# tylerlum/Vine_Robot_IsaacGymEnvs

Hardware: AMD Instinct MI355X
Metric: env-steps/sec Vine5LinkMovingBase 16384 envs per GPU (higher is better)
Workload: dtype f32 (env step, rollout inference); update: fp16 GEMM operands and backward-only saved activations (gates, saved cell states, dG, dh), f32 accumulate / recurrent state / heads / loss / optimiser, device-side GradScaler loss scaling (mixed_precision: True = the reference YAML's value, PY:53); rollout

## Files before the change

### vine_robot_isaacgymenvs_amd/csrc/ppo_kernels.hip

```cpp

#include <hip/hip_runtime.h>

#include <cstdio>
#include <cstdlib>

#include "../../include/vine.h"
#include "../../include/vine_ppo.h"
#include "vine_policy_head.h"
#include "vine_ppo_formulas.h"

namespace {

__device__ __forceinline__ float4 ld4(const float* p) { return *reinterpret_cast<const float4*>(p); }
__device__ __forceinline__ void st4(float* p, float4 v) { *reinterpret_cast<float4*>(p) = v; }

typedef unsigned short lp16_t;
typedef __attribute__((__vector_size__(2 * sizeof(float)))) float f32x2_hw;
#ifdef VINE_LP_BF16
typedef __bf16 lp16_hw;
#define VINE_LP16_NAME "bf16"
#define MFMA_LP16_BUILTIN __builtin_amdgcn_mfma_f32_16x16x32_bf16
#define DS_READ_TR16_B64 __builtin_amdgcn_ds_read_tr16_b64_v4bf16
typedef __bf16 lp16_tr_hw;
#define LP16_MAX 3.3895314e38f
// ... 286 lines not shown
    }
    __syncthreads();
    const int q = threadIdx.x & 15, rg = threadIdx.x >> 4;
    const int j = u0 + 4 * q;
    float bv[4][4];
#pragma unroll
    for (int g = 0; g < 4; ++g) {
        const float4 bb = ld4(bias + g * H + j);
        bv[g][0] = bb.x; bv[g][1] = bb.y; bv[g][2] = bb.z; bv[g][3] = bb.w;
    }
#pragma unroll
    for (int p = 0; p < 4; ++p) {
        const int r = rg + 16 * p;
        const long long b = (long long)blockIdx.x * 64 + r;
        const float keep = keep_pre[p], kn = kn_pre[p];
        float pre[4][4];
#pragma unroll
        for (int g = 0; g < 4; ++g) {
            const float4 a = *reinterpret_cast<const float4*>(&gt[r * GP + g * 64 + 4 * q]);
            pre[g][0] = a.x + bv[g][0]; pre[g][1] = a.y + bv[g][1]; pre[g][2] = a.z + bv[g][2]; pre[g][3] = a.w + bv[g][3];
            if (igates) {
                const float4 ig = ld4(igates + b * ig_stride + g * H + j);
                pre[g][0] += ig.x; pre[g][1] += ig.y; pre[g][2] += ig.z; pre[g][3] += ig.w;
            }
        }
        const float4 cp = cpre[p];
        const float cpv[4] = {cp.x, cp.y, cp.z, cp.w};
        float gi[4], gf[4], gg[4], go[4], cn[4], hn[4];
#pragma unroll
        for (int u = 0; u < 4; ++u)
            lstm_cell(pre[0][u], pre[1][u], pre[2][u], pre[3][u], keep * cpv[u], gi[u], gf[u], gg[u], go[u], cn[u], hn[u]);
        st4(c_out + b * H + j, make_float4(cn[0], cn[1], cn[2], cn[3]));
        st4(h_out + b * h_stride + j, make_float4(hn[0], hn[1], hn[2], hn[3]));
        if (hp_next) st4(hp_next + b * hp_stride + j, make_float4(kn * hn[0], kn * hn[1], kn * hn[2], kn * hn[3]));
        if (gates_act) {
            lp16_t* ga = gates_act + b * 4LL * H;
            st4(ga + 0 * H + j, make_float4(gi[0], gi[1], gi[2], gi[3]));
            st4(ga + 1 * H + j, make_float4(gf[0], gf[1], gf[2], gf[3]));
            st4(ga + 2 * H + j, make_float4(gg[0], gg[1], gg[2], gg[3]));
            st4(ga + 3 * H + j, make_float4(go[0], go[1], go[2], go[3]));
        }
    }
}

__device__ __forceinline__ float dpp_i2f(int x) { return __builtin_bit_cast(float, x); }
__device__ __forceinline__ int dpp_f2i(float x) { return __builtin_bit_cast(int, x); }
constexpr int SEQ_ROWS = 32;
constexpr int LDS_SKEW = 16;
constexpr int SEQ_FWD_NC = 11;
constexpr int SEQ_H = 256;
#ifndef SEQ_BWD_RING
#define SEQ_BWD_RING 8
#endif

__device__ __forceinline__ void seq_barrier() {
    asm volatile("s_waitcnt lgkmcnt(0)\n\ts_barrier" ::: "memory");
}

__global__ __launch_bounds__(256) void lstm_tile_weights_kernel(const lp16_t* __restrict__ src, long long ld, int H, int ksteps,
                                                                int nj, int transposed, lp16_t* __restrict__ dst) {
    const long long chunks = (long long)(H / 32) * ksteps * nj * 64;
    for (long long c = (long long)blockIdx.x * blockDim.x + threadIdx.x; c < chunks; c += (long long)gridDim.x * blockDim.x) {
        const int lane = (int)(c & 63);
        long long r = c >> 6;
        const int j = (int)(r % nj); r /= nj;
        const int kk = (int)(r % ksteps);
        const int w = (int)(r / ksteps);
        const int ut = nj == 8 ? (j & 1) : j, g = nj == 8 ? (j >> 1) : 0;
        const int unit = 32 * w + 8 * ((lane & 15) >> 2) + 4 * ut + (lane & 3);
        const int k0 = 32 * kk + 8 * (lane >> 4);
        uint4 v;
        if (!transposed) {
            v = *reinterpret_cast<const uint4*>(src + (long long)(g * H + unit) * ld + k0);
        } else {
            lp16_t e[8];
#pragma unroll
            for (int i = 0; i < 8; ++i) e[i] = src[(long long)(k0 + i) * ld + unit];
            v.x = e[0] | ((unsigned)e[1] << 16); v.y = e[2] | ((unsigned)e[3] << 16);
            v.z = e[4] | ((unsigned)e[5] << 16); v.w = e[6] | ((unsigned)e[7] << 16);
        }
        *reinterpret_cast<uint4*>(dst + c * 8) = v;
    }
}

typedef __attribute__((__vector_size__(4 * sizeof(unsigned)))) unsigned u32x4_t;
__device__ __forceinline__ uint4 seq_load_frag(__amdgpu_buffer_rsrc_t rsrc, int voffset, int soffset) {
    const u32x4_t v = __builtin_amdgcn_raw_buffer_load_b128(rsrc, voffset, soffset, 0);
    return make_uint4(v[0], v[1], v[2], v[3]);
}
__device__ __forceinline__ uint4 pack_lp16x8(const float (&v)[8]) {
    uint4 r;
    r.x = f2lp2(v[0], v[1]); r.y = f2lp2(v[2], v[3]); r.z = f2lp2(v[4], v[5]); r.w = f2lp2(v[6], v[7]);
    return r;
}

#ifdef SPLIT_TIMING
__device__ unsigned long long mlp_split_t[4096 * 16];
#endif
#if defined(SPLIT_TIMING) && defined(BWD_STAMPS)
#define BSTAMP(i)                                                                                                       \
    if ((threadIdx.x & 63) == 0) {                                                                                      \
        mlp_split_t[((blockIdx.x * 8 + (threadIdx.x >> 6)) & 4095) * 16 + 2 * (i)] = __builtin_amdgcn_s_memtime();      \
        mlp_split_t[((blockIdx.x * 8 + (threadIdx.x >> 6)) & 4095) * 16 + 2 * (i) + 1] = __builtin_amdgcn_s_memrealtime(); \
    }
#else
#define BSTAMP(i)
#endif
#ifdef SEQ_TIMING
__device__ unsigned long long seq_t[256 * 8 * 16];
#endif
template <int KS1, int RING, typename CT, typename HT, int NC>
__device__ __forceinline__ void lstm_seq_fwd_body(
    int T, long long B, const lp16_t* __restrict__ x, long long ldx, lp16_t* hp, long long hp_stride,
    const uint4* __restrict__ Wt, const float* __restrict__ bias, const float* __restrict__ c0,
    const unsigned char* __restrict__ done, HT* __restrict__ h_out, CT* __restrict__ c_all,
    lp16_t* __restrict__ gates, int ablate, float* __restrict__ c_last, const float* __restrict__ h0) {
    constexpr int H = SEQ_H, KSTEPS = KS1 + 8, KX = 32 * KS1, NF = KSTEPS * 8;
    constexpr int XP = KX + LDS_SKEW, HP = H + LDS_SKEW;
    static_assert(NF % RING == 0, "the ring must close on a step boundary");
    extern __shared__ __attribute__((aligned(16))) unsigned char seqf_lds[];
    float* bias_l = reinterpret_cast<float*>(seqf_lds);
    lp16_t (*hl)[SEQ_ROWS * HP] = reinterpret_cast<lp16_t (*)[SEQ_ROWS * HP]>(seqf_lds + 4 * H * sizeof(float));
    lp16_t (*xs)[SEQ_ROWS * XP] = reinterpret_cast<lp16_t (*)[SEQ_ROWS * XP]>(seqf_lds + 4 * H * sizeof(float) +
                                                                            2 * SEQ_ROWS * HP * sizeof(lp16_t));
    const int tid = threadIdx.x, lane = tid & 63;
    const int w = __builtin_amdgcn_readfirstlane(tid >> 6);
    const int col = lane & 15, lq = lane >> 4;
    const long long b0 = (long long)blockIdx.x * SEQ_ROWS;
    const int U0 = 32 * w + 8 * lq;
    const __amdgpu_buffer_rsrc_t wrsrc = __builtin_amdgcn_make_buffer_rsrc(
        const_cast<char*>(reinterpret_cast<const char*>(Wt) + (long long)w * NF * 1024), 0, NF * 1024, 0x00020000);
    const int wlane = lane * 16;
#define SEQ_WFRAG(f) seq_load_frag(wrsrc, wlane, (f) * 1024)
    uint4 ring[RING];
#pragma unroll
    for (int i = 0; i < RING; ++i) ring[i] = SEQ_WFRAG(i);
    static_assert(NC <= NF - RING && NC <= RING, "cached fragments are re-requested from the tail of the previous step only");
    uint4* wcache = reinterpret_cast<uint4*>(seqf_lds + 4 * H * sizeof(float) + 2 * SEQ_ROWS * HP * sizeof(lp16_t) +
                                             (size_t)T * SEQ_ROWS * XP * sizeof(lp16_t)) + (w * NC) * 64 + lane;
    {
        for (int p = tid; p < T * SEQ_ROWS * (KX / 8); p += 512) {
            const int tt = p / (SEQ_ROWS * (KX / 8)), q = p - tt * (SEQ_ROWS * (KX / 8));
            const int r = q / (KX / 8), c8 = q - r * (KX / 8);
            *reinterpret_cast<uint4*>(&xs[tt][r * XP + 8 * c8]) =
                *reinterpret_cast<const uint4*>(x + ((b0 + r) * T + tt) * ldx + 8 * c8);
        }
        for (int p = tid; p < SEQ_ROWS * (H / 8); p += 512) {
            const int r = p >> 5, c8 = p & 31;
            uint4 hv;
            if (h0) {
                const float keep0 = (done && done[(b0 + r) * T]) ? 0.0f : 1.0f;
                const float4 a = ld4(h0 + (b0 + r) * H + 8 * c8), b = ld4(h0 + (b0 + r) * H + 8 * c8 + 4);
                const float v[8] = {keep0 * a.x, keep0 * a.y, keep0 * a.z, keep0 * a.w, keep0 * b.x, keep0 * b.y, keep0 * b.z, keep0 * b.w};
                hv = pack_lp16x8(v);
                if (sizeof(HT) == 2) {
                    const float u8[8] = {a.x, a.y, a.z, a.w, b.x, b.y, b.z, b.w};
                    *reinterpret_cast<uint4*>(reinterpret_cast<lp16_t*>(h_out) + (b0 + r) * (T + 1) * H + 8 * c8) = pack_lp16x8(u8);
                } else {
                    *reinterpret_cast<uint4*>(hp + (b0 + r) * hp_stride + 8 * c8) = hv;
                }
            } else {
                hv = *reinterpret_cast<const uint4*>(hp + (b0 + r) * hp_stride + 8 * c8);
            }
            *reinterpret_cast<uint4*>(&hl[0][r * HP + 8 * c8]) = hv;
        }
        for (int p = tid; p < H; p += 512) st4(&bias_l[4 * p], ld4(bias + 4 * p));
    }
    float c[2][8];
    unsigned dmask[2];
#pragma unroll
    for (int rt = 0; rt < 2; ++rt) {
        const long long b = b0 + 16 * rt + col;
        const float4 a = ld4(c0 + b * H + U0), bb = ld4(c0 + b * H + U0 + 4);
        c[rt][0] = a.x; c[rt][1] = a.y; c[rt][2] = a.z; c[rt][3] = a.w;
        c[rt][4] = bb.x; c[rt][5] = bb.y; c[rt][6] = bb.z; c[rt][7] = bb.w;
        unsigned m = 0;
        if (done)
            for (int t = 0; t < T; ++t) m |= (done[b * T + t] ? 1u : 0u) << t;
        dmask[rt] = m;
    }
#pragma unroll 1
    for (int t = 0; t < T; ++t) {
#ifdef SEQ_TIMING
        if (lane == 0 && t < 4) seq_t[(blockIdx.x * 8 + w) * 16 + 4 * t + 0] = wall_clock64();
#endif
        if (t == 0) seq_barrier();
        const lp16_t* xb = xs[t];
        const lp16_t* hb = hl[t & 1];
        lp16_t* hnext = hl[(t + 1) & 1];
        const bool last = t == T - 1;
// ... 37 lines not shown
#endif
                    const int fn = (f + RING) % NF;
                    if (fn < NC && f + RING >= NF) ring[slot] = wcache[fn * 64];
                    else ring[slot] = SEQ_WFRAG(fn);
                }
                __builtin_amdgcn_sched_barrier(0);
            }
        }
#ifdef SEQ_TIMING
        if (lane == 0 && t < 4) seq_t[(blockIdx.x * 8 + w) * 16 + 4 * t + 2] = wall_clock64();
#endif
#pragma unroll
        for (int rt = 0; rt < 2; ++rt) {
            const long long b = b0 + 16 * rt + col;
            const float keep = ((dmask[rt] >> t) & 1u) ? 0.0f : 1.0f;
            const float kn = ((dmask[rt] >> (t + 1)) & 1u) ? 0.0f : 1.0f;
            CT* cp = c_all + ((long long)(t + 1) * B + b) * H + U0;
            float* cl = c_last + b * H + U0;
            HT* hpo = h_out + (sizeof(HT) == 2 ? b * (T + 1) + t + 1 : b * T + t) * H + U0;
            uint2 lo[6];
#pragma unroll
            for (int ut = 0; ut < 2; ++ut) {
                const float4 bi = *reinterpret_cast<const float4*>(&bias_l[0 * H + U0 + 4 * ut]);
                const float4 bf_ = *reinterpret_cast<const float4*>(&bias_l[1 * H + U0 + 4 * ut]);
                const float4 bg = *reinterpret_cast<const float4*>(&bias_l[2 * H + U0 + 4 * ut]);
                const float4 bo = *reinterpret_cast<const float4*>(&bias_l[3 * H + U0 + 4 * ut]);
                const float bv[4][4] = {{bi.x, bi.y, bi.z, bi.w}, {bf_.x, bf_.y, bf_.z, bf_.w}, {bg.x, bg.y, bg.z, bg.w},
                                        {bo.x, bo.y, bo.z, bo.w}};
                float gi[4], gf[4], gg[4], go[4], hn[4];
#pragma unroll
                for (int u = 0; u < 4; ++u)
                    lstm_cell(acc[0][ut][rt][u] + bv[0][u], acc[1][ut][rt][u] + bv[1][u], acc[2][ut][rt][u] + bv[2][u],
                              acc[3][ut][rt][u] + bv[3][u], keep * c[rt][4 * ut + u], gi[u], gf[u], gg[u], go[u],
                              c[rt][4 * ut + u], hn[u]);
                if (!(ablate & 1)) {
                    const float4 cv = make_float4(c[rt][4 * ut], c[rt][4 * ut + 1], c[rt][4 * ut + 2], c[rt][4 * ut + 3]);
                    if (sizeof(CT) == 2 && last) st4(cl + 4 * ut, cv);
                    else st4(cp + 4 * ut, cv);
                    if (sizeof(HT) == 4) st4(hpo + 4 * ut, make_float4(hn[0], hn[1], hn[2], hn[3]));
                }
                uint2 pk[6];
                pk[5] = make_uint2(f2lp2(hn[0], hn[1]), f2lp2(hn[2], hn[3]));
                pk[0] = make_uint2(f2lp2(gi[0], gi[1]), f2lp2(gi[2], gi[3]));
                pk[1] = make_uint2(f2lp2(gf[0], gf[1]), f2lp2(gf[2], gf[3]));
                pk[2] = make_uint2(f2lp2(gg[0], gg[1]), f2lp2(gg[2], gg[3]));
                pk[3] = make_uint2(f2lp2(go[0], go[1]), f2lp2(go[2], go[3]));
                pk[4] = make_uint2(f2lp2(kn * hn[0], kn * hn[1]), f2lp2(kn * hn[2], kn * hn[3]));
                if (ut == 0) {
#pragma unroll
                    for (int a = 0; a < 6; ++a) lo[a] = pk[a];
                } else {
                    if (sizeof(HT) == 2 && !(ablate & 1))
                        *reinterpret_cast<uint4*>(hpo) = make_uint4(lo[5].x, lo[5].y, pk[5].x, pk[5].y);
                    if (gates && !(ablate & 1)) {
                        lp16_t* ga = gates + ((long long)t * B + b) * 4 * H + U0;
#pragma unroll
                        for (int g = 0; g < 4; ++g)
                            *reinterpret_cast<uint4*>(ga + g * H) = make_uint4(lo[g].x, lo[g].y, pk[g].x, pk[g].y);
                    }
                    if (!last) {
                        const uint4 hm = make_uint4(lo[4].x, lo[4].y, pk[4].x, pk[4].y);
                        *reinterpret_cast<uint4*>(&hnext[(16 * rt + col) * HP + U0]) = hm;
                        if (sizeof(HT) == 4 && !(ablate & 1))
                            *reinterpret_cast<uint4*>(hp + b * hp_stride + (long long)(t + 1) * H + U0) = hm;
                    }
                }
            }
        }
#ifdef SEQ_TIMING
        if (lane == 0 && t < 4) seq_t[(blockIdx.x * 8 + w) * 16 + 4 * t + 3] = wall_clock64();
#endif
    }
}
template <int KS1, int RING, typename CT, typename HT, int NC>
__global__ __launch_bounds__(512) void lstm_seq_fwd_kernel(
    int T, long long B, const lp16_t* __restrict__ x, long long ldx, lp16_t* hp, long long hp_stride,
    const uint4* __restrict__ Wt, const float* __restrict__ bias, const float* __restrict__ c0,
    const unsigned char* __restrict__ done, HT* __restrict__ h_out, CT* __restrict__ c_all,
    lp16_t* __restrict__ gates, int ablate, float* __restrict__ c_last, const float* __restrict__ h0) {
    lstm_seq_fwd_body<KS1, RING, CT, HT, NC>(T, B, x, ldx, hp, hp_stride, Wt, bias, c0, done, h_out, c_all, gates, ablate, c_last,
                                             h0);
}

__device__ __forceinline__ float dpp_row_sum16(float v) {
    float s = v + dpp_i2f(__builtin_amdgcn_update_dpp(0, dpp_f2i(v), 0x111, 0xf, 0xf, true));
    s += dpp_i2f(__builtin_amdgcn_update_dpp(0, dpp_f2i(v), 0x112, 0xf, 0xf, true));
    s += dpp_i2f(__builtin_amdgcn_update_dpp(0, dpp_f2i(v), 0x113, 0xf, 0xf, true));
    s += dpp_i2f(__builtin_amdgcn_update_dpp(0, dpp_f2i(s), 0x114, 0xf, 0xe, true));
    s += dpp_i2f(__builtin_amdgcn_update_dpp(0, dpp_f2i(s), 0x118, 0xf, 0xc, true));
    return s;
}
__device__ __forceinline__ void unpack_lp16x8(uint4 r, float (&v)[8]) {
    unpack2(r.x, v[0], v[1]); unpack2(r.y, v[2], v[3]); unpack2(r.z, v[4], v[5]); unpack2(r.w, v[6], v[7]);
}

template <int RING, typename CT, typename GT>
__device__ __forceinline__ void lstm_seq_bwd_body(
    int T, long long B, const GT* __restrict__ g_out, const uint4* __restrict__ Wt, const lp16_t* __restrict__ gates,
    const CT* __restrict__ c_all, const float* __restrict__ c0, const unsigned char* __restrict__ done,
    lp16_t* __restrict__ dG, float* __restrict__ bias_partial, int ablate, const float* __restrict__ c_last) {
    constexpr int H = SEQ_H, K = 4 * H, KSTEPS = K / 32, NF = KSTEPS * 2;
    constexpr int PITCH = K + LDS_SKEW;
    static_assert(NF % RING == 0, "the ring must close on a step boundary");
    extern __shared__ __attribute__((aligned(16))) unsigned char seq_lds[];
    lp16_t (*dgl)[SEQ_ROWS * PITCH] = reinterpret_cast<lp16_t (*)[SEQ_ROWS * PITCH]>(seq_lds);
    const int tid = threadIdx.x, lane = tid & 63;
    const int w = __builtin_amdgcn_readfirstlane(tid >> 6);
    const int col = lane & 15, lq = lane >> 4;
    const long long b0 = (long long)blockIdx.x * SEQ_ROWS;
    const int U0 = 32 * w + 8 * lq;
    const __amdgpu_buffer_rsrc_t wrsrc = __builtin_amdgcn_make_buffer_rsrc(
        const_cast<char*>(reinterpret_cast<const char*>(Wt) + (long long)w * NF * 1024), 0, NF * 1024, 0x00020000);
    const int wlane = lane * 16;
    uint4 ring[RING];
#pragma unroll
    for (int i = 0; i < RING; ++i) ring[i] = SEQ_WFRAG(i);
    unsigned dmask[2];
    float dcarry[2][8], cnew[2][8], bsum[4][8];
#pragma unroll
    for (int rt = 0; rt < 2; ++rt) {
        const long long b = b0 + 16 * rt + col;
        unsigned m = 0;
        if (done)
            for (int t = 0; t < T; ++t) m |= (done[b * T + t] ? 1u : 0u) << t;
        dmask[rt] = m;
        float4 a, bb;
        if (sizeof(CT) == 2) { a = ld4(c_last + b * H + U0); bb = ld4(c_last + b * H + U0 + 4); }
        else { a = ld4(c_all + ((long long)T * B + b) * H + U0); bb = ld4(c_all + ((long long)T * B + b) * H + U0 + 4); }
        cnew[rt][0] = a.x; cnew[rt][1] = a.y; cnew[rt][2] = a.z; cnew[rt][3] = a.w;
        cnew[rt][4] = bb.x; cnew[rt][5] = bb.y; cnew[rt][6] = bb.z; cnew[rt][7] = bb.w;
#pragma unroll
        for (int e = 0; e < 8; ++e) dcarry[rt][e] = 0.0f;
    }
#pragma unroll
    for (int g = 0; g < 4; ++g)
#pragma unroll
        for (int e = 0; e < 8; ++e) bsum[g][e] = 0.0f;
    auto step = [&](const int t, auto first_c) __attribute__((always_inline)) {
        constexpr bool first = decltype(first_c)::value;
        float4 go4[2][2], cp4[2][2];
        uint4 gpk[2][4];
#define SEQ_BWD_LOAD(rt)                                                                                   \
        {                                                                                                  \
            const long long b_ = b0 + 16 * (rt) + col;                                                     \
            const GT* gp_ = g_out + (b_ * T + t) * H + U0;                                                 \
            go4[rt][0] = ld4(gp_); go4[rt][1] = ld4(gp_ + 4);                                              \
            if (t == 0) {                                                                                  \
                cp4[rt][0] = ld4(c0 + b_ * H + U0); cp4[rt][1] = ld4(c0 + b_ * H + U0 + 4);                \
            } else {                                                                                       \
                const CT* cpp_ = c_all + ((long long)t * B + b_) * H + U0;                                 \
                cp4[rt][0] = ld4(cpp_); cp4[rt][1] = ld4(cpp_ + 4);                                        \
            }                                                                                              \
            const lp16_t* ga_ = gates + ((long long)t * B + b_) * 4 * H + U0;                              \
            _Pragma("unroll") for (int g = 0; g < 4; ++g) gpk[rt][g] = *reinterpret_cast<const uint4*>(ga_ + g * H); \
        }
        SEQ_BWD_LOAD(0)
        f32x4_t acc[2][2];
#pragma unroll
        for (int ut = 0; ut < 2; ++ut)
#pragma unroll
            for (int rt = 0; rt < 2; ++rt) acc[ut][rt] = f32x4_t{0.0f, 0.0f, 0.0f, 0.0f};
        if (!first) {
            seq_barrier();
            const lp16_t* xb = dgl[(t + 1) & 1];
            if (t == T - 2) { BSTAMP(5) }
#pragma unroll
            for (int kk = 0; kk < KSTEPS; ++kk) {
                const lp16x8_t a0 = *reinterpret_cast<const lp16x8_t*>(xb + col * PITCH + 32 * kk + 8 * lq);
                const lp16x8_t a1 = *reinterpret_cast<const lp16x8_t*>(xb + (16 + col) * PITCH + 32 * kk + 8 * lq);
#pragma unroll
                for (int j = 0; j < 2; ++j) {
                    const int f = kk * 2 + j, slot = f % RING;
                    const lp16x8_t wf = __builtin_bit_cast(lp16x8_t, ring[slot]);
                    acc[j][0] = MFMA_LP16(wf, a0, acc[j][0]);
                    acc[j][1] = MFMA_LP16(wf, a1, acc[j][1]);
                    if (!(ablate & 2)) ring[slot] = SEQ_WFRAG((f + RING) % NF);
                    __builtin_amdgcn_sched_barrier(0);
                }
            }
            if (t == T - 2) { BSTAMP(6) }
        }
        lp16_t* dgn = dgl[t & 1];
        SEQ_BWD_LOAD(1)
#undef SEQ_BWD_LOAD
#pragma unroll
        for (int rt = 0; rt < 2; ++rt) {
            const long long b = b0 + 16 * rt + col;
            const float keep = ((dmask[rt] >> t) & 1u) ? 0.0f : 1.0f;
            const float keep_n = ((dmask[rt] >> (t + 1)) & 1u) ? 0.0f : 1.0f;
            lp16_t* dgp = dG + (b * T + t) * 4 * H + U0;
            uint2 lo[4];
#pragma unroll
            for (int ut = 0; ut < 2; ++ut) {
                float gi[4], gf[4], gg[4], go[4];
                const unsigned ia = ut ? gpk[rt][0].z : gpk[rt][0].x, ib = ut ? gpk[rt][0].w : gpk[rt][0].y;
                const unsigned fa = ut ? gpk[rt][1].z : gpk[rt][1].x, fb = ut ? gpk[rt][1].w : gpk[rt][1].y;
                const unsigned ga_ = ut ? gpk[rt][2].z : gpk[rt][2].x, gb_ = ut ? gpk[rt][2].w : gpk[rt][2].y;
                const unsigned oa = ut ? gpk[rt][3].z : gpk[rt][3].x, ob = ut ? gpk[rt][3].w : gpk[rt][3].y;
                unpack2(ia, gi[0], gi[1]); unpack2(ib, gi[2], gi[3]);
                unpack2(fa, gf[0], gf[1]); unpack2(fb, gf[2], gf[3]);
                unpack2(ga_, gg[0], gg[1]); unpack2(gb_, gg[2], gg[3]);
                unpack2(oa, go[0], go[1]); unpack2(ob, go[2], go[3]);
                const float gout[4] = {go4[rt][ut].x, go4[rt][ut].y, go4[rt][ut].z, go4[rt][ut].w};
                const float cp[4] = {cp4[rt][ut].x, cp4[rt][ut].y, cp4[rt][ut].z, cp4[rt][ut].w};
                float di[4], df[4], dg[4], dout[4];
#pragma unroll
                for (int u = 0; u < 4; ++u) {
                    const int e = 4 * ut + u;
                    float dh = gout[u];
                    if (!first) dh += keep_n * acc[ut][rt][u];
                    float dc = first ? 0.0f : keep_n * dcarry[rt][e];
                    if (!first) asm volatile("" : "+v"(dc));
                    lstm_cell_bwd(dh, dc, cnew[rt][e], keep * cp[u], gi[u], gf[u], gg[u], go[u], di[u], df[u], dg[u], dout[u],
                                  dcarry[rt][e]);
                    cnew[rt][e] = cp[u];
                    bsum[0][e] += di[u]; bsum[1][e] += df[u]; bsum[2][e] += dg[u]; bsum[3][e] += dout[u];
                }
                uint2 pk[4];
                pk[0] = make_uint2(f2lp2(di[0], di[1]), f2lp2(di[2], di[3]));
                pk[1] = make_uint2(f2lp2(df[0], df[1]), f2lp2(df[2], df[3]));
                pk[2] = make_uint2(f2lp2(dg[0], dg[1]), f2lp2(dg[2], dg[3]));
                pk[3] = make_uint2(f2lp2(dout[0], dout[1]), f2lp2(dout[2], dout[3]));
                if (ut == 0) {
#pragma unroll
                    for (int g = 0; g < 4; ++g) lo[g] = pk[g];
                } else {
                    lp16_t* row = dgn + (16 * rt + col) * PITCH + U0;
#pragma unroll
                    for (int g = 0; g < 4; ++g) {
                        const uint4 v = make_uint4(lo[g].x, lo[g].y, pk[g].x, pk[g].y);
                        if (!(ablate & 1)) *reinterpret_cast<uint4*>(dgp + g * H) = v;
                        if (t > 0) *reinterpret_cast<uint4*>(row + g * H) = v;
                    }
                }
            }
// ... 2601 lines not shown
    __syncthreads();
    if (threadIdx.x == 0) {
        const unsigned t = atomicAdd(ticket, 1u);
        is_last = t == gridDim.x - 1;
        if (is_last) *ticket = 0;
    }
    __syncthreads();
    if (is_last) {
        __threadfence();
        ppo_loss_finalize((int)gridDim.x, A, n, loss_partial, logstd, critic_coef, entropy_coef, bounds_coef, stats,
                          grad_logstd, grad_mu_bias, grad_value_bias, kl_out, logstd_grad_accum, S);
    }
}
template <int NH, int NP, typename DXT, typename XT>
__global__ __launch_bounds__(512) void ln_heads_loss_kernel(
    long long n, const XT* __restrict__ x, int xT, const float* __restrict__ gamma, const float* __restrict__ beta, float eps,
    const float* __restrict__ w, const float* __restrict__ wb, const float* __restrict__ logstd,
    const float* __restrict__ actions, const float* __restrict__ old_neglogp, const float* __restrict__ adv,
    const float* __restrict__ old_values, const float* __restrict__ returns, const float* old_mu, const float* old_sigma,
    float e_clip, int clip_value, float critic_coef, float entropy_coef, float bounds_coef, float soft_bound,
    float* __restrict__ heads, DXT* __restrict__ dx, float* __restrict__ ln_partial, float* loss_partial,
    float* __restrict__ stats, float* __restrict__ grad_logstd, float* __restrict__ grad_mu_bias,
    float* __restrict__ grad_value_bias, float* __restrict__ kl_out, float* __restrict__ logstd_grad_accum, float* mu_store,
    float* sigma_store, const float* __restrict__ loss_scale, float* __restrict__ found_inf, unsigned int* ticket,
    int defer) {
    __shared__ float red_s[8 * (2 + NH) * 256];
    __shared__ float lred_s[8 * PPO_LOSS_ROW];
    ln_heads_loss_body<NH, NP, DXT, XT>(red_s, lred_s, n, x, xT, gamma, beta, eps, w, wb, logstd, actions, old_neglogp, adv,
                                        old_values, returns, old_mu, old_sigma, e_clip, clip_value, critic_coef, entropy_coef,
                                        bounds_coef, soft_bound, heads, dx, ln_partial, loss_partial, stats, grad_logstd,
                                        grad_mu_bias, grad_value_bias, kl_out, logstd_grad_accum, mu_store, sigma_store,
                                        loss_scale, found_inf, ticket, defer);
}

struct TrunkPhasesArgs {
    long long B; int T;
    const lp16_t* x; long long ldx; const uint4* w_tiled; const float* bias; const float* c0; const float* h0;
    const unsigned char* done; lp16_t* h_out; lp16_t* c_all; lp16_t* gates; float* c_last; int ablate;
    const float* gamma; const float* beta; float eps; const float* w; const float* wb; const float* logstd;
    const float* actions; const float* old_neglogp; const float* adv; const float* old_values; const float* returns;
    const float* old_mu; const float* old_sigma; float e_clip; int clip_value; float critic_coef, entropy_coef, bounds_coef,
        soft_bound;
    float* heads; lp16_t* dx; float* ln_partial; float* loss_partial; float* stats; float* grad_logstd; float* grad_mu_bias;
    float* grad_value_bias; float* kl_out; float* logstd_grad_accum; float* mu_store; float* sigma_store;
    const float* loss_scale; float* found_inf;
    const uint4* w_hh_tiled; lp16_t* dG; float* bias_partial;
    const lp16_t* wt0; long long ldw0; const lp16_t* wt1; long long ldw1; const lp16_t* wt2; long long ldw2;
    const lp16_t* a3; long long a3_stride; const lp16_t* a2; const lp16_t* a1; float alpha;
    lp16_t* gz3; lp16_t* gz2; lp16_t* gz1; float* part3; float* part2; float* part1;
};
__global__ __launch_bounds__(512) void trunk_phases_kernel(const TrunkPhasesArgs a) {
    extern __shared__ __attribute__((aligned(16))) unsigned char trunk_lds[];
    TRUNK_STAMP(0)
    lstm_seq_fwd_body<3, 22, lp16_t, lp16_t, SEQ_FWD_NC>(a.T, a.B, a.x, a.ldx, nullptr, 0, a.w_tiled, a.bias, a.c0, a.done, a.h_out, a.c_all,
                                                 a.gates, a.ablate, a.c_last, a.h0);
    __syncthreads();
    TRUNK_STAMP(1)
    ln_heads_loss_body<3, 4, lp16_t, lp16_t>(reinterpret_cast<float*>(trunk_lds),
                                             reinterpret_cast<float*>(trunk_lds) + 8 * 5 * 256, a.B * a.T, a.h_out, a.T, a.gamma,
                                             a.beta, a.eps, a.w, a.wb, a.logstd, a.actions, a.old_neglogp, a.adv, a.old_values,
                                             a.returns, a.old_mu, a.old_sigma, a.e_clip, a.clip_value, a.critic_coef,
                                             a.entropy_coef, a.bounds_coef, a.soft_bound, a.heads, a.dx, a.ln_partial,
                                             a.loss_partial, a.stats, a.grad_logstd, a.grad_mu_bias, a.grad_value_bias, a.kl_out,
                                             a.logstd_grad_accum, a.mu_store, a.sigma_store, a.loss_scale, a.found_inf, nullptr,
                                             1 );
    __syncthreads();
    TRUNK_STAMP(2)
    lstm_seq_bwd_body<SEQ_BWD_RING, lp16_t, lp16_t>(a.T, a.B, a.dx, a.w_hh_tiled, a.gates, a.c_all, a.c0, a.done, a.dG,
                                                    a.bias_partial, a.ablate, a.c_last);
    __syncthreads();
    TRUNK_STAMP(3)
    mlp3_bwd_elu_mfma_body<64, 128, 256, 8, 8>(a.B * a.T, a.dG, 4 * SEQ_H, a.wt0, a.ldw0, a.wt1, a.ldw1, a.wt2, a.ldw2, a.a3,
                                              a.a3_stride, a.a2, a.a1, a.alpha, a.gz3, a.gz2, a.gz1, a.part3, a.part2, a.part1);
    TRUNK_STAMP(4)
}
#undef LHL_COL
#undef LHL_ROW

#define GRAD_SQNORM_MAX_PARTS 256
template <int CTRL, int ROW_MASK, int BANK_MASK>
__device__ __forceinline__ double dpp_f64(double v) {
    const unsigned long long b = __builtin_bit_cast(unsigned long long, v);
    const unsigned lo = (unsigned)__builtin_amdgcn_update_dpp(0, (int)(unsigned)b, CTRL, ROW_MASK, BANK_MASK, true);
    const unsigned hi = (unsigned)__builtin_amdgcn_update_dpp(0, (int)(unsigned)(b >> 32), CTRL, ROW_MASK, BANK_MASK, true);
    return __builtin_bit_cast(double, ((unsigned long long)hi << 32) | lo);
}
__device__ __forceinline__ double wave_sum_f64(double v) {
    double s = v + dpp_f64<0x111, 0xf, 0xf>(v);
    s += dpp_f64<0x112, 0xf, 0xf>(v);
    s += dpp_f64<0x113, 0xf, 0xf>(v);
    s += dpp_f64<0x114, 0xf, 0xe>(s);
    s += dpp_f64<0x118, 0xf, 0xc>(s);
    s += dpp_f64<0x142, 0xa, 0xf>(s);
    s += dpp_f64<0x143, 0xc, 0xf>(s);
    const unsigned long long b = __builtin_bit_cast(unsigned long long, s);
    const unsigned lo = (unsigned)__builtin_amdgcn_readlane((int)(unsigned)b, 63);
    const unsigned hi = (unsigned)__builtin_amdgcn_readlane((int)(unsigned)(b >> 32), 63);
    return __builtin_bit_cast(double, ((unsigned long long)hi << 32) | lo);
}

__global__ __launch_bounds__(256) void grad_sqnorm_kernel(long long n, const float* __restrict__ g,
                                                          double* __restrict__ partial) {
    __shared__ double ws[4];
    const long long n4 = n >> 2, stride = (long long)gridDim.x * 256;
    double a0 = 0.0, a1 = 0.0, a2 = 0.0, a3 = 0.0;
    for (long long i = (long long)blockIdx.x * 256 + threadIdx.x; i < n4; i += 2 * stride) {
        const bool more = i + stride < n4;
        const float4 x = ld4(g + 4 * i);
        const float4 y = more ? ld4(g + 4 * (i + stride)) : make_float4(0.0f, 0.0f, 0.0f, 0.0f);
        a0 = fma((double)x.x, (double)x.x, a0);
        a1 = fma((double)x.y, (double)x.y, a1);
        a2 = fma((double)x.z, (double)x.z, a2);
        a3 = fma((double)x.w, (double)x.w, a3);
        a0 = fma((double)y.x, (double)y.x, a0);
        a1 = fma((double)y.y, (double)y.y, a1);
        a2 = fma((double)y.z, (double)y.z, a2);
        a3 = fma((double)y.w, (double)y.w, a3);
    }
    if (blockIdx.x == 0 && (long long)threadIdx.x < (n & 3)) {
        const double x = (double)g[(n4 << 2) + threadIdx.x];
        a0 = fma(x, x, a0);
    }
    const double w = wave_sum_f64((a0 + a1) + (a2 + a3));
    if ((threadIdx.x & 63) == 0) ws[threadIdx.x >> 6] = w;
    __syncthreads();
    if (threadIdx.x == 0) partial[blockIdx.x] = (ws[0] + ws[1]) + (ws[2] + ws[3]);
// ... 1450 lines not shown
                           (size_t)8 * (64 + 128 + 256) * sizeof(float);
    const size_t lds = lds_lstm > lds_mlp ? lds_lstm : lds_mlp;
    if (!ensure_dyn_lds(reinterpret_cast<const void*>(&lstm_seq_bwd_mlp3_bwd_kernel<RING, lp16_t, lp16_t>), 160 * 1024))
        return VINE_ERR_DEVICE;
    hipLaunchKernelGGL((lstm_seq_bwd_mlp3_bwd_kernel<RING, lp16_t, lp16_t>), dim3((unsigned)(B / SEQ_ROWS)), dim3(512), lds,
                       (hipStream_t)stream, (int)T, (long long)B, (const lp16_t*)g_out, (const uint4*)w_hh_tiled,
                       (const lp16_t*)gates, (const lp16_t*)c_all, c0, done, (lp16_t*)dgates, bias_partial, seq_ablate(), c_last,
                       (const lp16_t*)wt0, (long long)ldw0, (const lp16_t*)wt1, (long long)ldw1, (const lp16_t*)wt2,
                       (long long)ldw2, (const lp16_t*)a3, (long long)a3_stride, (const lp16_t*)a2, (const lp16_t*)a1, alpha,
                       (lp16_t*)gz3, (lp16_t*)gz2, (lp16_t*)gz1, part3, part2, part1);
    return hipGetLastError() == hipSuccess ? VINE_OK : VINE_ERR_DEVICE;
}

int64_t vine_trunk_args_size(void) { return (int64_t)sizeof(VineTrunkArgs); }

int vine_trunk_phases(const VineTrunkArgs* p, void* stream) {
    if (!p) return VINE_ERR_INVALID_ARG;
    const VineTrunkArgs& q = *p;
    const void* need[] = {q.x, q.w_tiled, q.bias, q.c0, q.h0, q.h_out, q.c_all, q.gates, q.c_last, q.ln_gamma, q.ln_beta, q.w_heads,
                          q.b_heads, q.logstd, q.actions, q.old_neglogp, q.advantages, q.old_values, q.returns, q.old_mu,
                          q.old_sigma, q.heads, q.d_out, q.ln_partial, q.loss_partial, q.stats, q.grad_logstd, q.w_hh_tiled,
                          q.dgates, q.bias_partial, q.wt0, q.wt1, q.wt2, q.a3, q.a2, q.a1, q.gz3, q.gz2, q.gz1, q.part3, q.part2,
                          q.part1};
    for (const void* v : need)
        if (!v) return VINE_ERR_INVALID_ARG;
    if (q.B <= 0 || ((q.grad_mu_bias == nullptr) != (q.grad_value_bias == nullptr)) || ((q.mu_store == nullptr) != (q.sigma_store == nullptr)) ||
        (q.ldx & 7) || (q.ldw0 & 7) || (q.ldw1 & 7) || (q.ldw2 & 7) || (q.a3_stride & 7) || q.ldw0 < 4 * SEQ_H || q.ldw1 < 64 ||
        q.ldw2 < 128)
        return VINE_ERR_INVALID_ARG;
    const void* al16[] = {q.x, q.w_tiled, q.h_out, q.c_all, q.gates, q.d_out, q.w_hh_tiled, q.dgates, q.wt0, q.wt1, q.wt2, q.a3, q.a2,
                          q.a1, q.gz3, q.gz2, q.gz1, q.c0, q.h0, q.c_last, q.bias};
    for (const void* v : al16)
        if ((uintptr_t)v & 15) return VINE_ERR_INVALID_ARG;
    const long long n = q.B * q.T;
    if (q.T != 4 || (q.B % SEQ_ROWS) || q.ldx < 96 || n / 128 > VINE_PPO_LOSS_BLOCKS) return VINE_ERR_UNSUPPORTED;
    TrunkPhasesArgs a;
    a.B = q.B; a.T = (int)q.T;
    a.x = (const lp16_t*)q.x; a.ldx = q.ldx; a.w_tiled = (const uint4*)q.w_tiled; a.bias = q.bias; a.c0 = q.c0; a.h0 = q.h0;
    a.done = q.done; a.h_out = (lp16_t*)q.h_out; a.c_all = (lp16_t*)q.c_all; a.gates = (lp16_t*)q.gates; a.c_last = q.c_last;
    a.ablate = seq_ablate();
    a.gamma = q.ln_gamma; a.beta = q.ln_beta; a.eps = q.ln_eps; a.w = q.w_heads; a.wb = q.b_heads; a.logstd = q.logstd;
    a.actions = q.actions; a.old_neglogp = q.old_neglogp; a.adv = q.advantages; a.old_values = q.old_values; a.returns = q.returns;
    a.old_mu = q.old_mu; a.old_sigma = q.old_sigma; a.e_clip = q.e_clip; a.clip_value = q.clip_value; a.critic_coef = q.critic_coef;
    a.entropy_coef = q.entropy_coef; a.bounds_coef = q.bounds_coef; a.soft_bound = q.soft_bound;
    a.heads = q.heads; a.dx = (lp16_t*)q.d_out; a.ln_partial = q.ln_partial; a.loss_partial = q.loss_partial; a.stats = q.stats;
    a.grad_logstd = q.grad_logstd; a.grad_mu_bias = q.grad_mu_bias; a.grad_value_bias = q.grad_value_bias; a.kl_out = q.kl_out;
    a.logstd_grad_accum = q.logstd_grad_accum; a.mu_store = q.mu_store; a.sigma_store = q.sigma_store; a.loss_scale = q.loss_scale;
    a.found_inf = q.found_inf;
    a.w_hh_tiled = (const uint4*)q.w_hh_tiled; a.dG = (lp16_t*)q.dgates; a.bias_partial = q.bias_partial;
    a.wt0 = (const lp16_t*)q.wt0; a.ldw0 = q.ldw0; a.wt1 = (const lp16_t*)q.wt1; a.ldw1 = q.ldw1; a.wt2 = (const lp16_t*)q.wt2;
    a.ldw2 = q.ldw2; a.a3 = (const lp16_t*)q.a3; a.a3_stride = q.a3_stride; a.a2 = (const lp16_t*)q.a2; a.a1 = (const lp16_t*)q.a1;
    a.alpha = q.alpha; a.gz3 = (lp16_t*)q.gz3; a.gz2 = (lp16_t*)q.gz2; a.gz1 = (lp16_t*)q.gz1; a.part3 = q.part3; a.part2 = q.part2;
    a.part1 = q.part1;
    const size_t lds = 160 * 1024;
    if (!ensure_dyn_lds(reinterpret_cast<const void*>(&trunk_phases_kernel), lds)) return VINE_ERR_DEVICE;
    hipLaunchKernelGGL(trunk_phases_kernel, dim3((unsigned)(q.B / SEQ_ROWS)), dim3(512), lds, (hipStream_t)stream, a);
    return hipGetLastError() == hipSuccess ? VINE_OK : VINE_ERR_DEVICE;
}

int vine_linear_bwd_elu_mfma(int64_t n, int64_t N, int64_t K, const void* G, int64_t ldg, const void* Wt, int64_t ldw,
                             const void* a, int64_t a_stride, float alpha, void* gz, int64_t gz_stride, float* partial,
                             void* stream) {
    if (n <= 0 || N <= 0 || K <= 0 || !G || !Wt || !a || !gz || (ldg & 7) || (ldw & 7) || (a_stride & 3) || (gz_stride & 3))
        return VINE_ERR_INVALID_ARG;
    if ((n & 63) || (N & 63) || (K != 64 && K != 128 && K != 256 && K != 512 && K != 1024)) return VINE_ERR_UNSUPPORTED;
    const dim3 grid((unsigned)(n / 64), (unsigned)(N / 64)), block(256);
    if (K >= 512) {
        hipStream_t s2 = (hipStream_t)stream;
        if (K == 512)
            hipLaunchKernelGGL(linear_bwd_elu_mfma_chunked_kernel<4>, grid, block, 0, s2, (long long)n, (int)N,
                               (const lp16_t*)G, (long long)ldg, (const lp16_t*)Wt, (long long)ldw, (const lp16_t*)a,
                               (long long)a_stride, alpha, (lp16_t*)gz, (long long)gz_stride, partial);
        else
            hipLaunchKernelGGL(linear_bwd_elu_mfma_chunked_kernel<8>, grid, block, 0, s2, (long long)n, (int)N,
                               (const lp16_t*)G, (long long)ldg, (const lp16_t*)Wt, (long long)ldw, (const lp16_t*)a,
                               (long long)a_stride, alpha, (lp16_t*)gz, (long long)gz_stride, partial);
        return hipGetLastError() == hipSuccess ? VINE_OK : VINE_ERR_DEVICE;
    }
    size_t lds = (size_t)64 * (K + 8) * sizeof(lp16_t);
    if (lds < 64 * 65 * sizeof(float)) lds = 64 * 65 * sizeof(float);
    hipStream_t s = (hipStream_t)stream;
#define VINE_LINB_MFMA(KS)                                                                                             \
    hipLaunchKernelGGL(linear_bwd_elu_mfma_kernel<KS>, grid, block, lds, s, (long long)n, (int)N, (const lp16_t*)G,    \
                       (long long)ldg, (const lp16_t*)Wt, (long long)ldw, (const lp16_t*)a, (long long)a_stride, alpha,  \
                       (lp16_t*)gz, (long long)gz_stride, partial)
    switch (K / 32) {
        case 2: VINE_LINB_MFMA(2); break;
        case 4: VINE_LINB_MFMA(4); break;
        case 8: VINE_LINB_MFMA(8); break;
        default: return VINE_ERR_UNSUPPORTED;
    }
#undef VINE_LINB_MFMA
    return hipGetLastError() == hipSuccess ? VINE_OK : VINE_ERR_DEVICE;
}

int vine_lstm_cell_backward(int64_t B, int64_t H, const float* g_out, int64_t g_stride, const float* g_rec,
                            const float* dc_next, const uint8_t* done_next, int64_t done_next_stride,
                            const void* gates_act, const float* c_new, const float* c_prev, const uint8_t* done,
                            int64_t done_stride, void* dgates, int64_t dg_stride, float* dc_prev,
                            float* bias_partial, const float* bias_partial_prev, int32_t dgates_bf16, void* stream) {
    if (B <= 0 || H <= 0 || (H & 3) || (g_stride & 3) || (dg_stride & 3) || !g_out || !gates_act || !c_new || !c_prev ||
        !dgates || !dc_prev)
        return VINE_ERR_INVALID_ARG;
    const int threads = 256;
    if (bias_partial && (H > 1024 || threads % (int)(H / 4) != 0)) return VINE_ERR_UNSUPPORTED;
    const int blocks = bias_partial ? VINE_PPO_PARTIAL_BLOCKS : grid_for(B * (H / 4), threads);
    if (dgates_bf16)
// ... 804 lines not shown
```

Baseline: 27.69 million.

## Stash last-step LSTM gates in LDS for the fused trunk backward

In the fused trunk kernel, the forward LSTM pass no longer writes the last timestep's gate activations to global memory. It keeps them in the LDS region that held the weight-fragment cache. The backward pass then reads that first (reverse) step's gates straight from LDS instead of global memory. To keep the stash intact, the double-buffered dG LDS parity is flipped, and static asserts check that the loss phase and the dgl buffers stay below the stash offset. This removes one global round trip per block on the critical start of the backward recurrence, but it depends on carefully reasoned LDS aliasing across phases.

```diff
diff --git a/vine_robot_isaacgymenvs_amd/csrc/ppo_kernels.hip b/vine_robot_isaacgymenvs_amd/csrc/ppo_kernels.hip
--- a/vine_robot_isaacgymenvs_amd/csrc/ppo_kernels.hip
+++ b/vine_robot_isaacgymenvs_amd/csrc/ppo_kernels.hip
@@ -362,6 +362,12 @@
 #ifndef SEQ_BWD_RING
 #define SEQ_BWD_RING 8
 #endif
+constexpr int seq_fwd_rows_bytes(int T, int KS1) {
+    return 4 * SEQ_H * (int)sizeof(float) + 2 * SEQ_ROWS * (SEQ_H + LDS_SKEW) * 2 + T * SEQ_ROWS * (32 * KS1 + LDS_SKEW) * 2;
+}
+constexpr int SEQ_DGL_BYTES = SEQ_ROWS * (4 * SEQ_H + LDS_SKEW) * 2;
+constexpr int TRUNK_LDS_BYTES = 160 * 1024;
+constexpr int TRUNK_STASH_OFF = seq_fwd_rows_bytes(4, 3);
 
 __device__ __forceinline__ void seq_barrier() {
     asm volatile("s_waitcnt lgkmcnt(0)\n\ts_barrier" ::: "memory");
@@ -419,7 +425,7 @@
 #ifdef SEQ_TIMING
 __device__ unsigned long long seq_t[256 * 8 * 16];
 #endif
-template <int KS1, int RING, typename CT, typename HT, int NC>
+template <int KS1, int RING, typename CT, typename HT, int NC, bool STASH = false>
 __device__ __forceinline__ void lstm_seq_fwd_body(
     int T, long long B, const lp16_t* __restrict__ x, long long ldx, lp16_t* hp, long long hp_stride,
     const uint4* __restrict__ Wt, const float* __restrict__ bias, const float* __restrict__ c0,
@@ -446,6 +452,7 @@
 #pragma unroll
     for (int i = 0; i < RING; ++i) ring[i] = SEQ_WFRAG(i);
     static_assert(NC <= NF - RING && NC <= RING, "cached fragments are re-requested from the tail of the previous step only");
+    static_assert(!STASH || NC >= 8, "the gates of the last step take 8 slots of the wave's cache region");
     uint4* wcache = reinterpret_cast<uint4*>(seqf_lds + 4 * H * sizeof(float) + 2 * SEQ_ROWS * HP * sizeof(lp16_t) +
                                              (size_t)T * SEQ_ROWS * XP * sizeof(lp16_t)) + (w * NC) * 64 + lane;
     {
@@ -589,7 +596,10 @@
                 } else {
                     if (sizeof(HT) == 2 && !(ablate & 1))
                         *reinterpret_cast<uint4*>(hpo) = make_uint4(lo[5].x, lo[5].y, pk[5].x, pk[5].y);
-                    if (gates && !(ablate & 1)) {
+                    if (STASH && last) {
+#pragma unroll
+                        for (int g = 0; g < 4; ++g) wcache[(4 * rt + g) * 64] = make_uint4(lo[g].x, lo[g].y, pk[g].x, pk[g].y);
+                    } else if (gates && !(ablate & 1)) {
                         lp16_t* ga = gates + ((long long)t * B + b) * 4 * H + U0;
 #pragma unroll
                         for (int g = 0; g < 4; ++g)
@@ -631,7 +641,7 @@
     unpack2(r.x, v[0], v[1]); unpack2(r.y, v[2], v[3]); unpack2(r.z, v[4], v[5]); unpack2(r.w, v[6], v[7]);
 }
 
-template <int RING, typename CT, typename GT>
+template <int RING, typename CT, typename GT, int STASH = 0>
 __device__ __forceinline__ void lstm_seq_bwd_body(
     int T, long long B, const GT* __restrict__ g_out, const uint4* __restrict__ Wt, const lp16_t* __restrict__ gates,
     const CT* __restrict__ c_all, const float* __restrict__ c0, const unsigned char* __restrict__ done,
@@ -641,6 +651,8 @@
     static_assert(NF % RING == 0, "the ring must close on a step boundary");
     extern __shared__ __attribute__((aligned(16))) unsigned char seq_lds[];
     lp16_t (*dgl)[SEQ_ROWS * PITCH] = reinterpret_cast<lp16_t (*)[SEQ_ROWS * PITCH]>(seq_lds);
+    static_assert(sizeof(lp16_t) * SEQ_ROWS * PITCH == SEQ_DGL_BYTES, "dgl buffer size");
+    static_assert(STASH == 0 || (STASH >= SEQ_DGL_BYTES && STASH % 16 == 0), "the first step's dG rows (dgl[0]) end below the stash");
     const int tid = threadIdx.x, lane = tid & 63;
     const int w = __builtin_amdgcn_readfirstlane(tid >> 6);
     const int col = lane & 15, lq = lane >> 4;
@@ -649,6 +661,8 @@
     const __amdgpu_buffer_rsrc_t wrsrc = __builtin_amdgcn_make_buffer_rsrc(
         const_cast<char*>(reinterpret_cast<const char*>(Wt) + (long long)w * NF * 1024), 0, NF * 1024, 0x00020000);
     const int wlane = lane * 16;
+    const uint4* stash = reinterpret_cast<const uint4*>(seq_lds + STASH) + (w * SEQ_FWD_NC) * 64 + lane;
+    (void)stash;
     uint4 ring[RING];
 #pragma unroll
     for (int i = 0; i < RING; ++i) ring[i] = SEQ_WFRAG(i);
@@ -688,8 +702,12 @@
                 const CT* cpp_ = c_all + ((long long)t * B + b_) * H + U0;                                 \
                 cp4[rt][0] = ld4(cpp_); cp4[rt][1] = ld4(cpp_ + 4);                                        \
             }                                                                                              \
-            const lp16_t* ga_ = gates + ((long long)t * B + b_) * 4 * H + U0;                              \
-            _Pragma("unroll") for (int g = 0; g < 4; ++g) gpk[rt][g] = *reinterpret_cast<const uint4*>(ga_ + g * H); \
+            if (first && STASH > 0) {                                                                      \
+                _Pragma("unroll") for (int g = 0; g < 4; ++g) gpk[rt][g] = stash[(4 * (rt) + g) * 64];         \
+            } else {                                                                                       \
+                const lp16_t* ga_ = gates + ((long long)t * B + b_) * 4 * H + U0;                          \
+                _Pragma("unroll") for (int g = 0; g < 4; ++g) gpk[rt][g] = *reinterpret_cast<const uint4*>(ga_ + g * H); \
+            }                                                                                              \
         }
         SEQ_BWD_LOAD(0)
         f32x4_t acc[2][2];
@@ -699,7 +717,7 @@
             for (int rt = 0; rt < 2; ++rt) acc[ut][rt] = f32x4_t{0.0f, 0.0f, 0.0f, 0.0f};
         if (!first) {
             seq_barrier();
-            const lp16_t* xb = dgl[(t + 1) & 1];
+            const lp16_t* xb = dgl[t & 1];
             if (t == T - 2) { BSTAMP(5) }
 #pragma unroll
             for (int kk = 0; kk < KSTEPS; ++kk) {
@@ -717,7 +735,7 @@
             }
             if (t == T - 2) { BSTAMP(6) }
         }
-        lp16_t* dgn = dgl[t & 1];
+        lp16_t* dgn = dgl[(t + 1) & 1];
         SEQ_BWD_LOAD(1)
 #undef SEQ_BWD_LOAD
 #pragma unroll
@@ -3425,10 +3443,12 @@
 __global__ __launch_bounds__(512) void trunk_phases_kernel(const TrunkPhasesArgs a) {
     extern __shared__ __attribute__((aligned(16))) unsigned char trunk_lds[];
     TRUNK_STAMP(0)
-    lstm_seq_fwd_body<3, 22, lp16_t, lp16_t, SEQ_FWD_NC>(a.T, a.B, a.x, a.ldx, nullptr, 0, a.w_tiled, a.bias, a.c0, a.done, a.h_out, a.c_all,
-                                                 a.gates, a.ablate, a.c_last, a.h0);
+    lstm_seq_fwd_body<3, 22, lp16_t, lp16_t, SEQ_FWD_NC, true>(a.T, a.B, a.x, a.ldx, nullptr, 0, a.w_tiled, a.bias, a.c0, a.done, a.h_out,
+                                                       a.c_all, a.gates, a.ablate, a.c_last, a.h0);
     __syncthreads();
     TRUNK_STAMP(1)
+    static_assert((8 * 5 * 256 + 8 * PPO_LOSS_ROW) * (int)sizeof(float) <= TRUNK_STASH_OFF, "the loss phase stays below the stashed gates");
+    static_assert(TRUNK_STASH_OFF + 8 * SEQ_FWD_NC * 1024 <= TRUNK_LDS_BYTES, "the forward phase's weight caches fit");
     ln_heads_loss_body<3, 4, lp16_t, lp16_t>(reinterpret_cast<float*>(trunk_lds),
                                              reinterpret_cast<float*>(trunk_lds) + 8 * 5 * 256, a.B * a.T, a.h_out, a.T, a.gamma,
                                              a.beta, a.eps, a.w, a.wb, a.logstd, a.actions, a.old_neglogp, a.adv, a.old_values,
@@ -3439,12 +3459,13 @@
                                              1 );
     __syncthreads();
     TRUNK_STAMP(2)
-    lstm_seq_bwd_body<SEQ_BWD_RING, lp16_t, lp16_t>(a.T, a.B, a.dx, a.w_hh_tiled, a.gates, a.c_all, a.c0, a.done, a.dG,
-                                                    a.bias_partial, a.ablate, a.c_last);
+    lstm_seq_bwd_body<SEQ_BWD_RING, lp16_t, lp16_t, TRUNK_STASH_OFF>(a.T, a.B, a.dx, a.w_hh_tiled, a.gates, a.c_all, a.c0, a.done,
+                                                                     a.dG, a.bias_partial, a.ablate, a.c_last);
     __syncthreads();
     TRUNK_STAMP(3)
-    mlp3_bwd_elu_mfma_body<64, 128, 256, 8, 8>(a.B * a.T, a.dG, 4 * SEQ_H, a.wt0, a.ldw0, a.wt1, a.ldw1, a.wt2, a.ldw2, a.a3,
-                                              a.a3_stride, a.a2, a.a1, a.alpha, a.gz3, a.gz2, a.gz1, a.part3, a.part2, a.part1);
+    mlp3_bwd_elu_mfma_body<64, 128, 256, 8, 8>(a.B * a.T, a.dG, 4 * SEQ_H, a.wt0, a.ldw0, a.wt1, a.ldw1, a.wt2, a.ldw2,
+                                                      a.a3, a.a3_stride, a.a2, a.a1, a.alpha, a.gz3, a.gz2, a.gz1, a.part3,
+                                                      a.part2, a.part1);
     TRUNK_STAMP(4)
 }
 #undef LHL_COL
@@ -5001,7 +5022,7 @@
     a.ldw2 = q.ldw2; a.a3 = (const lp16_t*)q.a3; a.a3_stride = q.a3_stride; a.a2 = (const lp16_t*)q.a2; a.a1 = (const lp16_t*)q.a1;
     a.alpha = q.alpha; a.gz3 = (lp16_t*)q.gz3; a.gz2 = (lp16_t*)q.gz2; a.gz1 = (lp16_t*)q.gz1; a.part3 = q.part3; a.part2 = q.part2;
     a.part1 = q.part1;
-    const size_t lds = 160 * 1024;
+    const size_t lds = TRUNK_LDS_BYTES;
     if (!ensure_dyn_lds(reinterpret_cast<const void*>(&trunk_phases_kernel), lds)) return VINE_ERR_DEVICE;
     hipLaunchKernelGGL(trunk_phases_kernel, dim3((unsigned)(q.B / SEQ_ROWS)), dim3(512), lds, (hipStream_t)stream, a);
     return hipGetLastError() == hipSuccess ? VINE_OK : VINE_ERR_DEVICE;
```

Result: no change. 27.96 million (median of 6 runs) (+1.0%).
